# jhbastek/PhysicsInformedDiffusionModels

Hardware: AMD Instinct MI355X
Metric: training samples/sec (UNet+PDE-residual step), 64x64 Darcy (higher is better)
Workload: dtype f32

## Files before the change

physicsinformeddiffusionmodels_amd/csrc/k_attn.hip:

```cpp
#include "pidm_launch.h"

namespace pidm {

static const int DH = 32;

__device__ __forceinline__ float fexp(float x) { return __expf(x); }

__global__ void __launch_bounds__(256) la_kstats_kernel(const float* __restrict__ qkv, int N, int HD, int nseg,
                                                        float* __restrict__ kpart, float* __restrict__ kstat) {
  __shared__ float sm[4][64], ssum[4][64];
  const int b = blockIdx.y, seg = blockIdx.z, tid = threadIdx.x, cl = tid & 63, rl = tid >> 6;
  const int j = blockIdx.x * 64 + cl;
  const int per = (N + nseg - 1) / nseg;
  const int n_lo = seg * per, n_hi = (n_lo + per < N) ? n_lo + per : N;
  float m = -3.0e38f, s = 0.f;
  if (j < HD) {
    const float* base = qkv + (size_t)b * N * 3 * HD + HD + j;
    int n = n_lo + rl;
    for (; n + 28 < n_hi; n += 32) {
      float v[8];
#pragma unroll
      for (int u = 0; u < 8; ++u) v[u] = base[(size_t)(n + 4 * u) * 3 * HD];
      float gm = v[0];
#pragma unroll
// ... 700 lines not shown
    for (int it = 0; it < 4; ++it) {
      const f32x4 v = *reinterpret_cast<const f32x4*>(tb + (trow + 8 * it) * kLaTileLd + tcol);
      *reinterpret_cast<f32x4*>(orow + (size_t)(trow + 8 * it) * 3 * HD + tcol) = v;
    }
  }
}

static const int kLaDkvLds = 32 * 33 + 96;
__global__ void __launch_bounds__(256, 3) la_bwd_dkdv_kernel(const float* __restrict__ qkv, const float* __restrict__ kstat,
                                                             const float* __restrict__ dctx, const float* __restrict__ rowdot,
                                                             float* __restrict__ dqkv, int N, int heads) {
  HIP_DYNAMIC_SHARED(float, sm)
  const int HD = heads * DH;
  const int tid = threadIdx.x, lane = tid & 63, wave = tid >> 6, half = lane >> 5, l31 = lane & 31;
  const size_t pblk = (size_t)blockIdx.x * 128;
  const int b = (int)(pblk / N);
  const size_t pa = pblk + wave * 32 + l31;
  const float invN = 1.f / (float)N;
  for (int i = tid; i < heads * 1024; i += 256)
    sm[(i >> 10) * kLaDkvLds + ((i & 1023) >> 5) * 33 + (i & 31)] = dctx[(size_t)b * heads * 1024 + i];
  for (int i = tid; i < heads * 32; i += 256) {
    float* hs = sm + (i >> 5) * kLaDkvLds + 1056;
    hs[i & 31] = rowdot[(size_t)b * heads * 32 + i];
    hs[32 + (i & 31)] = kstat[((size_t)b * HD + i) * 2];
    hs[64 + (i & 31)] = kstat[((size_t)b * HD + i) * 2 + 1];
  }
  __syncthreads();
  float* tb = sm + heads * kLaDkvLds + wave * (32 * kLaTileLd);
  const float* rowK = qkv + pa * 3 * HD + HD;
  f32x4 n_k[4], n_v[4], n_k4[4];
#pragma unroll
  for (int j = 0; j < 4; ++j) {
    n_k[j] = *reinterpret_cast<const f32x4*>(rowK + 16 * half + 4 * j);
    n_v[j] = *reinterpret_cast<const f32x4*>(rowK + HD + 16 * half + 4 * j);
    n_k4[j] = *reinterpret_cast<const f32x4*>(rowK + 8 * j + 4 * half);
  }
  for (int h = 0; h < heads; ++h) {
    const float* sd = sm + h * kLaDkvLds;
    const float* srd = sd + 1056;
    const float* skm = srd + 32;
    const float* skis = srd + 64;
    f32x4 a_k[4], a_v[4], k4[4];
#pragma unroll
    for (int j = 0; j < 4; ++j) { a_k[j] = n_k[j]; a_v[j] = n_v[j]; k4[j] = n_k4[j]; }
    if (h + 1 < heads) {
      const float* rn = rowK + (h + 1) * DH;
#pragma unroll
      for (int j = 0; j < 4; ++j) {
        n_k[j] = *reinterpret_cast<const f32x4*>(rn + 16 * half + 4 * j);
        n_v[j] = *reinterpret_cast<const f32x4*>(rn + HD + 16 * half + 4 * j);
        n_k4[j] = *reinterpret_cast<const f32x4*>(rn + 8 * j + 4 * half);
      }
    }
    f32x16 acc2, acc3;
    for (int r = 0; r < 16; ++r) { acc2[r] = 0.f; acc3[r] = 0.f; }
#pragma unroll
    for (int j = 0; j < 4; ++j) {
#pragma unroll
      for (int c = 0; c < 4; ++c) {
        const int kk = 16 * half + 4 * j + c;
        acc2 = __builtin_amdgcn_mfma_f32_32x32x2f32(sd[l31 * 33 + kk], a_v[j][c], acc2, 0, 0, 0);
        const float pB = fexp(a_k[j][c] - skm[kk]) * skis[kk];
        acc3 = __builtin_amdgcn_mfma_f32_32x32x2f32(sd[kk * 33 + l31], pB, acc3, 0, 0, 0);
      }
    }
    f32x4 o_k[4], o_v[4];
#pragma unroll
    for (int j = 0; j < 4; ++j) {
#pragma unroll
      for (int c = 0; c < 4; ++c) {
        const int d = 8 * j + 4 * half + c;
        const float P = fexp(k4[j][c] - skm[d]) * skis[d];
        o_k[j][c] = P * (acc2[4 * j + c] * invN - srd[d]);
        o_v[j][c] = acc3[4 * j + c] * invN;
      }
    }
    float* ok = dqkv + (pblk + wave * 32) * 3 * HD + HD + h * DH;
    const int trow = lane >> 3, tcol = 4 * (lane & 7);
#pragma unroll
    for (int which = 0; which < 2; ++which) {
      __builtin_amdgcn_wave_barrier();
#pragma unroll
      for (int j = 0; j < 4; ++j) *reinterpret_cast<f32x4*>(tb + l31 * kLaTileLd + 8 * j + 4 * half) = which ? o_v[j] : o_k[j];
      __builtin_amdgcn_wave_barrier();
#pragma unroll
      for (int it = 0; it < 4; ++it) {
        const f32x4 v = *reinterpret_cast<const f32x4*>(tb + (trow + 8 * it) * kLaTileLd + tcol);
        *reinterpret_cast<f32x4*>(ok + (size_t)(trow + 8 * it) * 3 * HD + which * HD + tcol) = v;
      }
    }
  }
}

template <bool BWD>
__global__ void __launch_bounds__(256) mid_attn_kernel(const float* __restrict__ qkv, const float* __restrict__ dO,
                                                       float* __restrict__ out,
                                                       int N, int heads, float scale) {
  HIP_DYNAMIC_SHARED(float, smem)
  float (*sq)[33] = reinterpret_cast<float (*)[33]>(smem);
  float (*sk)[33] = reinterpret_cast<float (*)[33]>(smem + (size_t)N * 33);
  float (*sv)[33] = reinterpret_cast<float (*)[33]>(smem + (size_t)2 * N * 33);
  float (*sdo)[33] = reinterpret_cast<float (*)[33]>(smem + (size_t)3 * N * 33);
  float* sS_ = smem + (size_t)4 * N * 33;
  float* sdS_ = sS_ + (size_t)N * (N + 1);
  const int LS = N + 1;
#define sS(i, j) sS_[(i) * LS + (j)]
#define sdS(i, j) sdS_[(i) * LS + (j)]
  const int HD = heads * DH;
  const int bh = blockIdx.x, b = bh / heads, h = bh % heads, tid = threadIdx.x;
  for (int e = tid; e < N * 32; e += 256) {
    const int n = e >> 5, d = e & 31;
    const float* row = qkv + ((size_t)b * N + n) * 3 * HD + h * DH + d;
    sq[n][d] = row[0] * scale;
    sk[n][d] = row[HD];
    sv[n][d] = row[2 * HD];
    if (BWD) sdo[n][d] = dO[((size_t)b * N + n) * HD + h * DH + d];
  }
  __syncthreads();
  for (int e = tid; e < N * N; e += 256) {
    const int i = e / N, j = e % N;
    float s = 0.f;
#pragma unroll
    for (int d = 0; d < 32; ++d) s = fmaf(sq[i][d], sk[j][d], s);
    sS(i, j) = s;
  }
  __syncthreads();
  if (tid < N) {
    float m = -3.0e38f;
    for (int j = 0; j < N; ++j) m = fmaxf(m, sS(tid, j));
    float s = 0.f;
    for (int j = 0; j < N; ++j) {
      const float ex = fexp(sS(tid, j) - m);
      sS(tid, j) = ex;
      s += ex;
    }
    const float inv = 1.f / s;
    for (int j = 0; j < N; ++j) sS(tid, j) *= inv;
  }
  __syncthreads();
  if (!BWD) {
    for (int e = tid; e < N * 32; e += 256) {
      const int i = e >> 5, d = e & 31;
      float o = 0.f;
      for (int j = 0; j < N; ++j) o = fmaf(sS(i, j), sv[j][d], o);
      out[((size_t)b * N + i) * HD + h * DH + d] = o;
    }
    return;
  }
  for (int e = tid; e < N * 32; e += 256) {
    const int j = e >> 5, d = e & 31;
    float o = 0.f;
    for (int i = 0; i < N; ++i) o = fmaf(sS(i, j), sdo[i][d], o);
    out[((size_t)b * N + j) * 3 * HD + 2 * HD + h * DH + d] = o;
  }
  __syncthreads();
  for (int e = tid; e < N * N; e += 256) {
    const int i = e / N, j = e % N;
    float s = 0.f;
#pragma unroll
    for (int d = 0; d < 32; ++d) s = fmaf(sdo[i][d], sv[j][d], s);
    sdS(i, j) = s;
  }
  __syncthreads();
  if (tid < N) {
    float dot = 0.f;
    for (int j = 0; j < N; ++j) dot = fmaf(sdS(tid, j), sS(tid, j), dot);
    for (int j = 0; j < N; ++j) sdS(tid, j) = sS(tid, j) * (sdS(tid, j) - dot);
  }
  __syncthreads();
  for (int e = tid; e < N * 32; e += 256) {
    const int i = e >> 5, d = e & 31;
    float a = 0.f, c = 0.f;
    for (int j = 0; j < N; ++j) {
      a = fmaf(sdS(i, j), sk[j][d], a);
      c = fmaf(sdS(j, i), sq[j][d], c);
    }
    out[((size_t)b * N + i) * 3 * HD + h * DH + d] = a * scale;
    out[((size_t)b * N + i) * 3 * HD + HD + h * DH + d] = c;
  }
}

#undef sS
#undef sdS

template <bool BWD>
__global__ void __launch_bounds__(256) mid_attn64_kernel(const float* __restrict__ qkv, const float* __restrict__ dO,
                                                         float* __restrict__ out, int heads, float scale) {
  constexpr int N = 64, LS = 65;
  HIP_DYNAMIC_SHARED(float, smem)
  float (*sq)[33] = reinterpret_cast<float (*)[33]>(smem);
  float (*sk)[33] = reinterpret_cast<float (*)[33]>(smem + (size_t)N * 33);
  float (*sv)[33] = reinterpret_cast<float (*)[33]>(smem + (size_t)2 * N * 33);
  float (*sdo)[33] = reinterpret_cast<float (*)[33]>(smem + (size_t)3 * N * 33);
  float* sS_ = smem + (size_t)4 * N * 33;
  float* sdS_ = sS_ + (size_t)N * LS;
  const int HD = heads * DH;
  const int bh = blockIdx.x, b = bh / heads, h = bh % heads, tid = threadIdx.x;
  const int lane = tid & 63, half = lane >> 5, l31 = lane & 31, wave = __builtin_amdgcn_readfirstlane(tid >> 6);
  for (int e = tid; e < N * 32; e += 256) {
    const int n = e >> 5, d = e & 31;
    const float* row = qkv + ((size_t)b * N + n) * 3 * HD + h * DH + d;
    sq[n][d] = row[0] * scale;
    sk[n][d] = row[HD];
    sv[n][d] = row[2 * HD];
    if (BWD) sdo[n][d] = dO[((size_t)b * N + n) * HD + h * DH + d];
  }
  __syncthreads();
  const int ti = wave >> 1, tj = wave & 1;
  {
    f32x16 acc;
    for (int r = 0; r < 16; ++r) acc[r] = 0.f;
#pragma unroll
    for (int s2 = 0; s2 < 16; ++s2)
      acc = __builtin_amdgcn_mfma_f32_32x32x2f32(sq[32 * ti + l31][2 * s2 + half], sk[32 * tj + l31][2 * s2 + half], acc, 0, 0, 0);
#pragma unroll
    for (int r = 0; r < 16; ++r) sS_[(32 * ti + (r & 3) + 8 * (r >> 2) + 4 * half) * LS + 32 * tj + l31] = acc[r];
  }
  __syncthreads();
  {
    const int row = tid >> 2, c0 = (tid & 3) * 16;
    float* pr = sS_ + row * LS + c0;
    float m = pr[0];
#pragma unroll
    for (int j = 1; j < 16; ++j) m = fmaxf(m, pr[j]);
    m = fmaxf(m, pidm_quad_xor1(m));
    m = fmaxf(m, pidm_quad_xor2(m));
    float ex[16], sum = 0.f;
#pragma unroll
    for (int j = 0; j < 16; ++j) { ex[j] = fexp(pr[j] - m); sum += ex[j]; }
    sum += pidm_quad_xor1(sum);
    sum += pidm_quad_xor2(sum);
    const float inv = 1.f / sum;
#pragma unroll
    for (int j = 0; j < 16; ++j) pr[j] = ex[j] * inv;
  }
  __syncthreads();
  if (!BWD) {
    if (wave < 2) {
      f32x16 acc;
      for (int r = 0; r < 16; ++r) acc[r] = 0.f;
#pragma unroll 8
      for (int s2 = 0; s2 < 32; ++s2)
        acc = __builtin_amdgcn_mfma_f32_32x32x2f32(sS_[(32 * wave + l31) * LS + 2 * s2 + half], sv[2 * s2 + half][l31], acc, 0, 0, 0);
#pragma unroll
      for (int r = 0; r < 16; ++r)
        out[((size_t)b * N + 32 * wave + (r & 3) + 8 * (r >> 2) + 4 * half) * HD + h * DH + l31] = acc[r];
    }
    return;
  }
  {
    f32x16 acc;
    for (int r = 0; r < 16; ++r) acc[r] = 0.f;
#pragma unroll
    for (int s2 = 0; s2 < 16; ++s2)
      acc = __builtin_amdgcn_mfma_f32_32x32x2f32(sdo[32 * ti + l31][2 * s2 + half], sv[32 * tj + l31][2 * s2 + half], acc, 0, 0, 0);
#pragma unroll
    for (int r = 0; r < 16; ++r) sdS_[(32 * ti + (r & 3) + 8 * (r >> 2) + 4 * half) * LS + 32 * tj + l31] = acc[r];
  }
  if (wave < 2) {
    f32x16 acc;
    for (int r = 0; r < 16; ++r) acc[r] = 0.f;
#pragma unroll 8
    for (int s2 = 0; s2 < 32; ++s2)
      acc = __builtin_amdgcn_mfma_f32_32x32x2f32(sS_[(2 * s2 + half) * LS + 32 * wave + l31], sdo[2 * s2 + half][l31], acc, 0, 0, 0);
#pragma unroll
    for (int r = 0; r < 16; ++r)
      out[((size_t)b * N + 32 * wave + (r & 3) + 8 * (r >> 2) + 4 * half) * 3 * HD + 2 * HD + h * DH + l31] = acc[r];
  }
  __syncthreads();
  {
    const int row = tid >> 2, c0 = (tid & 3) * 16;
    const float* pp = sS_ + row * LS + c0;
    float* pd = sdS_ + row * LS + c0;
    float dot = 0.f;
#pragma unroll
    for (int j = 0; j < 16; ++j) dot = fmaf(pd[j], pp[j], dot);
    dot += pidm_quad_xor1(dot);
    dot += pidm_quad_xor2(dot);
#pragma unroll
    for (int j = 0; j < 16; ++j) pd[j] = pp[j] * (pd[j] - dot);
  }
  __syncthreads();
  {
    const int t = wave & 1;
    f32x16 acc;
    for (int r = 0; r < 16; ++r) acc[r] = 0.f;
    if (wave < 2) {
#pragma unroll 8
      for (int s2 = 0; s2 < 32; ++s2)
        acc = __builtin_amdgcn_mfma_f32_32x32x2f32(sdS_[(32 * t + l31) * LS + 2 * s2 + half], sk[2 * s2 + half][l31], acc, 0, 0, 0);
    } else {
#pragma unroll 8
      for (int s2 = 0; s2 < 32; ++s2)
        acc = __builtin_amdgcn_mfma_f32_32x32x2f32(sdS_[(2 * s2 + half) * LS + 32 * t + l31], sq[2 * s2 + half][l31], acc, 0, 0, 0);
    }
    const float f = wave < 2 ? scale : 1.f;
    const size_t col = (wave < 2 ? 0 : HD) + h * DH + l31;
#pragma unroll
    for (int r = 0; r < 16; ++r)
      out[((size_t)b * N + 32 * t + (r & 3) + 8 * (r >> 2) + 4 * half) * 3 * HD + col] = acc[r] * f;
  }
}

static int la_nsplit(int N) {
  int ns = N / 512;
  if (ns < 1) ns = 1;
  if (ns > 8) ns = 8;
  return ns;
}
static int la_kseg(int N) {
  int s = N / 256;
  if (s < 1) s = 1;
  if (s > 16) s = 16;
  return s;
}
size_t la_scratch_floats(int B, int N, int heads) {
  const size_t a = (size_t)B * la_kseg(N) * heads * DH * 2, b = (size_t)B * heads * la_nsplit(N) * 1024;
  return a + b + (size_t)heads * DH * 128 + 64;
}

int launch_la_forward(const float* qkv, float* kstat, float* ctx, float* attn, float* qstat, int B, int N, int heads,
                      float* scratch, hipStream_t st) {
  const int HD = heads * DH;
  const float scale = 0.17677669529663687f;
  const int nseg = la_kseg(N), NS = la_nsplit(N);
  float* kpart = scratch;
  float* dpart = scratch + (size_t)B * nseg * HD * 2;
  hipLaunchKernelGGL(la_kstats_kernel, dim3(cdiv(HD, 64), B, nseg), dim3(256), 0, st, qkv, N, HD, nseg, kpart, nseg == 1 ? kstat : nullptr);
  PIDM_CHECK_LAUNCH("la_kstats_kernel");
  if (nseg > 1) {
    hipLaunchKernelGGL(la_kstats_final_kernel, dim3(cdiv(B * HD, 256)), dim3(256), 0, st, kpart, B, HD, nseg, kstat);
    PIDM_CHECK_LAUNCH("la_kstats_final_kernel");
  }
  hipLaunchKernelGGL(HIP_KERNEL_NAME(la_nreduce_kernel<0>), dim3(B * heads, NS), dim3(256), 0, st, qkv, kstat, nullptr, nullptr,
                     dpart, N, heads, scale, NS == 1 ? ctx : nullptr, nullptr, 1.f / (float)N);
  PIDM_CHECK_LAUNCH("la_context");
  if (NS > 1) {
    hipLaunchKernelGGL(HIP_KERNEL_NAME(la_nreduce_final_kernel<0>), dim3(B * heads), dim3(256), 0, st, dpart, nullptr, ctx, nullptr, NS,
                       1.f / (float)N);
    PIDM_CHECK_LAUNCH("la_context_final");
  }
  const size_t npix = (size_t)B * N;
  if (N % 32 == 0)
    hipLaunchKernelGGL(HIP_KERNEL_NAME(la_out_kernel<true>), dim3((unsigned)((npix + 127) / 128), (npix + 127) / 128 < 1024 ? heads : 1), dim3(256), 0, st, qkv, ctx, attn,
                       qstat, N, heads, npix, scale);
  else
    hipLaunchKernelGGL(HIP_KERNEL_NAME(la_out_kernel<false>), dim3((unsigned)((npix + 127) / 128), (npix + 127) / 128 < 1024 ? heads : 1), dim3(256), 0, st, qkv, ctx, attn,
                       qstat, N, heads, npix, scale);
  PIDM_CHECK_LAUNCH("la_out_kernel");
  return 0;
}

int launch_la_backward(const float* qkv, const float* kstat, const float* qstat, const float* ctx, const float* dA, float* dctx,
                       float* rowdot, float* dqkv, int B, int N, int heads, float* scratch, hipStream_t st) {
  const float scale = 0.17677669529663687f;
  const int NS = la_nsplit(N);
  float* dpart = scratch;
  hipLaunchKernelGGL(HIP_KERNEL_NAME(la_nreduce_kernel<1>), dim3(B * heads, NS), dim3(256), 0, st, qkv, qstat, dA, ctx, dpart, N, heads,
                     scale, NS == 1 ? dctx : nullptr, rowdot, 1.f);
  PIDM_CHECK_LAUNCH("la_dctx");
  if (NS > 1) {
    hipLaunchKernelGGL(HIP_KERNEL_NAME(la_nreduce_final_kernel<1>), dim3(B * heads), dim3(256), 0, st, dpart, ctx, dctx, rowdot, NS, 1.f);
    PIDM_CHECK_LAUNCH("la_dctx_final");
  }
  if (N % 32 == 0 && N >= 64) {
    const size_t npix = (size_t)B * N;
    int ppb = N % 128 == 0 ? 128 : (N % 64 == 0 ? 64 : 32);
    (void)npix;
    if (const char* pe = knob("PIDM_LA_PPB")) { const int v = atoi(pe); if ((v == 32 || v == 64 || v == 128) && N % v == 0) ppb = v; }
    PIDM_PROF_NAME("la_bwd_pix_mfma_kernel");
    hipLaunchKernelGGL(la_bwd_pix_mfma_kernel, dim3((unsigned)((size_t)B * N / ppb), heads), dim3(2 * ppb), 0, st, qkv, kstat, qstat, ctx,
                       dctx, rowdot, dA, dqkv, N, heads, scale, ppb);
  } else {
    hipLaunchKernelGGL(la_bwd_pix_kernel, dim3(cdiv(N, 256), B * heads), dim3(256), 0, st, qkv, kstat, qstat, ctx, dctx, rowdot,
                       dA, dqkv, N, heads, scale);
  }
  PIDM_CHECK_LAUNCH("la_bwd_pix_kernel");
  return 0;
}

bool la_fused_ok(int N, int heads, int Cout, int ld_dy) {
  const bool off = knob("PIDM_NO_LA_FUSED") != nullptr;
  return !off && N % 128 == 0 && (Cout == 32 || Cout == 64 || Cout == 128) && (ld_dy & 3) == 0 && heads >= 1 && heads <= 14;
}
int launch_la_forward_fused(const float* qkv, float* kstat, float* ctx, float* qstat, const float* w_out, const float* bias,
                            const float* resid, float* y, int Cout, int B, int N, int heads, float* scratch, hipStream_t st) {
  if (!la_fused_ok(N, heads, Cout, Cout)) return fail("fused attention forward: N=%d Cout=%d not eligible", N, Cout);
  const int HD = heads * DH;
  const float scale = 0.17677669529663687f;
  const int nseg = la_kseg(N), NS = la_nsplit(N);
  float* kpart = scratch;
  float* dpart = scratch + (size_t)B * nseg * HD * 2;
  hipLaunchKernelGGL(la_kstats_kernel, dim3(cdiv(HD, 64), B, nseg), dim3(256), 0, st, qkv, N, HD, nseg, kpart, nseg == 1 ? kstat : nullptr);
  PIDM_CHECK_LAUNCH("la_kstats_kernel");
  if (nseg > 1) {
    hipLaunchKernelGGL(la_kstats_final_kernel, dim3(cdiv(B * HD, 256)), dim3(256), 0, st, kpart, B, HD, nseg, kstat);
    PIDM_CHECK_LAUNCH("la_kstats_final_kernel");
  }
  hipLaunchKernelGGL(HIP_KERNEL_NAME(la_nreduce_kernel<0>), dim3(B * heads, NS), dim3(256), 0, st, qkv, kstat, nullptr, nullptr,
                     dpart, N, heads, scale, NS == 1 ? ctx : nullptr, nullptr, 1.f / (float)N);
  PIDM_CHECK_LAUNCH("la_context");
  if (NS > 1) {
    hipLaunchKernelGGL(HIP_KERNEL_NAME(la_nreduce_final_kernel<0>), dim3(B * heads), dim3(256), 0, st, dpart, nullptr, ctx, nullptr, NS,
                       1.f / (float)N);
    PIDM_CHECK_LAUNCH("la_context_final");
  }
  float* wt = dpart + (size_t)B * heads * NS * 1024;
  hipLaunchKernelGGL(la_wt_kernel, dim3(cdiv(Cout * HD, 256)), dim3(256), 0, st, w_out, wt, Cout, HD);
  PIDM_CHECK_LAUNCH("la_wt_kernel");
  const dim3 grid((unsigned)((size_t)B * N / 128));
  if (Cout == 32)
    hipLaunchKernelGGL(HIP_KERNEL_NAME(la_out_proj_kernel<1>), grid, dim3(256), 0, st, qkv, ctx, wt, bias, resid, y, qstat, N, heads, scale);
  else if (Cout == 64)
    hipLaunchKernelGGL(HIP_KERNEL_NAME(la_out_proj_kernel<2>), grid, dim3(256), 0, st, qkv, ctx, wt, bias, resid, y, qstat, N, heads, scale);
  else
    hipLaunchKernelGGL(HIP_KERNEL_NAME(la_out_proj_kernel<4>), grid, dim3(256), 0, st, qkv, ctx, wt, bias, resid, y, qstat, N, heads, scale);
  PIDM_CHECK_LAUNCH("la_out_proj_kernel");
  return 0;
}

bool la_fused_pays(int B, int N) {
  const char* mw = knob("PIDM_LA_FUSED_MIN_WGS");
  const long min_wgs = mw ? atol(mw) : 256;
  return (long)B * N / 128 >= min_wgs;
}
size_t la_fused_scratch_floats(int B, int N, int heads, int Cout) {
  return (size_t)B * heads * la_nsplit(N) * (Cout / 32) * 1024 + 64;
}
int launch_la_backward_fused(const float* qkv, const float* kstat, const float* qstat, const float* ctx, const float* dy, int ld_dy,
                             const float* w_out, int Cout, float* dctx, float* rowdot, float* dqkv, float* dwpart, int B, int N,
                             int heads, float* scratch, hipStream_t st) {
  if (!la_fused_ok(N, heads, Cout, ld_dy)) return fail("fused attention backward: N=%d Cout=%d not eligible", N, Cout);
  const float scale = 0.17677669529663687f;
  const int NS = la_nsplit(N);
  float* gpart = scratch;
  const dim3 grid(B * heads, NS);
#define PIDM_LA_G(NT_)                                                                                                        \
  {                                                                                                                           \
    hipLaunchKernelGGL(HIP_KERNEL_NAME(la_g_kernel<NT_>), grid, dim3(256), 0, st, qkv, qstat, dy, ld_dy, gpart, N, heads, scale); \
    PIDM_CHECK_LAUNCH("la_g_kernel");                                                                                         \
    hipLaunchKernelGGL(HIP_KERNEL_NAME(la_g_final_kernel<NT_>), dim3(B * heads), dim3(256), 0, st, gpart, ctx, w_out, dctx,    \
                       rowdot, dwpart, NS, heads);                                                                            \
    PIDM_CHECK_LAUNCH("la_g_final_kernel");                                                                                   \
  }
  if (Cout == 32) PIDM_LA_G(1)
  else if (Cout == 64) PIDM_LA_G(2)
  else PIDM_LA_G(4)
#undef PIDM_LA_G
  const dim3 gridp((unsigned)((size_t)B * N / 128));
  static bool attr_done = false;
  if (!attr_done) {
    (void)hipFuncSetAttribute(reinterpret_cast<const void*>(&la_bwd_dq_kernel), hipFuncAttributeMaxDynamicSharedMemorySize, 96 * 1024);
    (void)hipFuncSetAttribute(reinterpret_cast<const void*>(&la_bwd_dkdv_kernel), hipFuncAttributeMaxDynamicSharedMemorySize, 96 * 1024);
    attr_done = true;
  }
  hipLaunchKernelGGL(la_bwd_dq_kernel, gridp, dim3(256), ((size_t)heads * 1056 + 4 * 32 * kLaTileLd) * sizeof(float), st, qkv, qstat, ctx, dy, ld_dy, w_out, Cout,
                     dqkv, N, heads, scale);
  PIDM_CHECK_LAUNCH("la_bwd_dq_kernel");
  hipLaunchKernelGGL(la_bwd_dkdv_kernel, gridp, dim3(256), ((size_t)heads * kLaDkvLds + 4 * 32 * kLaTileLd) * sizeof(float), st, qkv, kstat, dctx, rowdot, dqkv, N,
                     heads);
  PIDM_CHECK_LAUNCH("la_bwd_dkdv_kernel");
  return 0;
}

int launch_mid_attn(const float* qkv, const float* dO, float* out, int B, int N, int heads, bool bwd, hipStream_t st) {
  if (N > 64) return fail("mid attention: %d tokens > 64", N);
  const float scale = 0.17677669529663687f;
  const size_t lds = ((size_t)4 * N * 33 + (size_t)2 * N * (N + 1)) * sizeof(float);
  static bool attr_done = false;
  if (!attr_done) {
    (void)hipFuncSetAttribute(reinterpret_cast<const void*>(&mid_attn_kernel<true>), hipFuncAttributeMaxDynamicSharedMemorySize, 96 * 1024);
    (void)hipFuncSetAttribute(reinterpret_cast<const void*>(&mid_attn_kernel<false>), hipFuncAttributeMaxDynamicSharedMemorySize, 96 * 1024);
    attr_done = true;
  }
  const bool mfma_off = [] { const char* e = knob("PIDM_MID_ATTN_MFMA"); return e && !atoi(e); }();
  if (N == 64 && !mfma_off) {
    static bool attr64 = false;
    if (!attr64) {
      (void)hipFuncSetAttribute(reinterpret_cast<const void*>(&mid_attn64_kernel<true>), hipFuncAttributeMaxDynamicSharedMemorySize, 96 * 1024);
      (void)hipFuncSetAttribute(reinterpret_cast<const void*>(&mid_attn64_kernel<false>), hipFuncAttributeMaxDynamicSharedMemorySize, 96 * 1024);
      attr64 = true;
    }
    if (bwd) hipLaunchKernelGGL(HIP_KERNEL_NAME(mid_attn64_kernel<true>), dim3(B * heads), dim3(256), lds, st, qkv, dO, out, heads, scale);
    else hipLaunchKernelGGL(HIP_KERNEL_NAME(mid_attn64_kernel<false>), dim3(B * heads), dim3(256), lds, st, qkv, dO, out, heads, scale);
    PIDM_CHECK_LAUNCH("mid_attn64_kernel");
    return 0;
  }
  if (bwd)
    hipLaunchKernelGGL(HIP_KERNEL_NAME(mid_attn_kernel<true>), dim3(B * heads), dim3(256), lds, st, qkv, dO, out, N, heads, scale);
  else
    hipLaunchKernelGGL(HIP_KERNEL_NAME(mid_attn_kernel<false>), dim3(B * heads), dim3(256), lds, st, qkv, dO, out, N, heads, scale);
  PIDM_CHECK_LAUNCH("mid_attn_kernel");
  return 0;
}

}

extern "C" size_t pidm_linear_attention_ws(int B, int N, int heads) {
  return ((size_t)B * heads * (1024 + 32) + pidm::la_scratch_floats(B, N, heads)) * sizeof(float);
}
extern "C" int pidm_linear_attention_forward(const float* qkv, float* out, float* kstat, float* ctx, float* qstat, int B, int N,
                                             int heads, void* workspace, void* stream) {
  if (!qkv || !out || !kstat || !ctx || !qstat || !workspace || B < 1 || N < 1 || heads < 1)
    return pidm::fail("linear attention: bad arguments");
  float* scratch = reinterpret_cast<float*>(workspace) + (size_t)B * heads * (1024 + 32);
  return pidm::launch_la_forward(qkv, kstat, ctx, out, qstat, B, N, heads, scratch, reinterpret_cast<hipStream_t>(stream));
}
extern "C" int pidm_linear_attention_backward(const float* qkv, const float* kstat, const float* qstat, const float* ctx,
                                              const float* d_out, float* dqkv, int B, int N, int heads, void* workspace,
                                              void* stream) {
  if (!qkv || !kstat || !qstat || !ctx || !d_out || !dqkv || !workspace || B < 1 || N < 1 || heads < 1)
    return pidm::fail("linear attention backward: bad arguments");
  float* dctx = reinterpret_cast<float*>(workspace);
  float* rowdot = dctx + (size_t)B * heads * 1024;
  float* scratch = rowdot + (size_t)B * heads * 32;
  return pidm::launch_la_backward(qkv, kstat, qstat, ctx, d_out, dctx, rowdot, dqkv, B, N, heads, scratch,
                                  reinterpret_cast<hipStream_t>(stream));
}
extern "C" size_t pidm_linear_attention_out_backward_ws(int B, int N, int heads, int Cout) {
  return ((size_t)B * heads * (1024 + 32) + (size_t)B * Cout * heads * 32 + pidm::la_fused_scratch_floats(B, N, heads, Cout)) *
         sizeof(float);
}
extern "C" int pidm_linear_attention_out_backward(const float* qkv, const float* kstat, const float* qstat, const float* ctx,
                                                  const float* d_y, int ld_dy, const float* w_out, int Cout, float* dqkv,
                                                  float* dw_out, int B, int N, int heads, void* workspace, void* stream) {
  if (!qkv || !kstat || !qstat || !ctx || !d_y || !w_out || !dqkv || !dw_out || !workspace || B < 1)
    return pidm::fail("fused attention backward: bad arguments");
  const int HD = heads * 32;
  float* dctx = reinterpret_cast<float*>(workspace);
  float* rowdot = dctx + (size_t)B * heads * 1024;
  float* dwpart = rowdot + (size_t)B * heads * 32;
  float* scratch = dwpart + (size_t)B * Cout * HD;
  hipStream_t st = reinterpret_cast<hipStream_t>(stream);
  if (pidm::launch_la_backward_fused(qkv, kstat, qstat, ctx, d_y, ld_dy, w_out, Cout, dctx, rowdot, dqkv, dwpart, B, N, heads,
                                     scratch, st))
    return -1;
  return pidm::launch_split_reduce(dwpart, dw_out, nullptr, nullptr, B, Cout, HD, 1, Cout, HD, st);
}
extern "C" int pidm_linear_attention_out_forward(const float* qkv, const float* w_out, const float* bias, const float* residual,
                                                 float* y, int Cout, float* kstat, float* ctx, float* qstat, int B, int N,
                                                 int heads, void* workspace, void* stream) {
  if (!qkv || !w_out || !y || !kstat || !ctx || !qstat || !workspace || B < 1) return pidm::fail("fused attention forward: bad arguments");
  float* scratch = reinterpret_cast<float*>(workspace) + (size_t)B * heads * (1024 + 32);
  return pidm::launch_la_forward_fused(qkv, kstat, ctx, qstat, w_out, bias, residual, y, Cout, B, N, heads, scratch,
                                       reinterpret_cast<hipStream_t>(stream));
}
```

Baseline: 7933.

## Fuse linear-attention forward and backward into single per-head LDS-resident kernels

For small spatial sizes (N between 64 and 256, multiple of 32), forward and backward linear attention each run as one kernel per (batch, head). The kernel stages K/V (or Q/K/dA) into LDS and computes key stats, context, query softmax and output with MFMA inside one block. This replaces the chain of separate stats, reduce, finalize and output launches and their global scratch round-trips. In exchange, parallelism drops to B*heads blocks that need large dynamic LDS, which can limit occupancy. The backward kernel also no longer writes dctx and rowdot to global memory.

```diff
diff --git a/physicsinformeddiffusionmodels_amd/csrc/k_attn.hip b/physicsinformeddiffusionmodels_amd/csrc/k_attn.hip
--- a/physicsinformeddiffusionmodels_amd/csrc/k_attn.hip
+++ b/physicsinformeddiffusionmodels_amd/csrc/k_attn.hip
@@ -1026,6 +1026,330 @@
   }
 }
 
+__device__ __forceinline__ int la_one_swz(int row, int piece) { return row * 32 + 4 * (piece ^ ((row >> 1) & 7)); }
+template <bool SWZ>
+__device__ __forceinline__ void la_one_stage(const float* __restrict__ src, size_t ld, float* __restrict__ dst, int N, int wave,
+                                             int nw, int lane) {
+  for (int c = wave; c < N / 8; c += nw) {
+    const int row = 8 * c + (lane >> 3);
+    const int piece = SWZ ? ((lane & 7) ^ ((row >> 1) & 7)) : (lane & 7);
+    pidm_glds_b128(src + (size_t)row * ld + 4 * piece, dst + 256 * c);
+  }
+}
+#ifdef PIDM_HAVE_ROW_SHL
+__device__ __forceinline__ float la_half_sum(float x) {
+  for (int off = 1; off < 32; off <<= 1) x += __shfl_xor(x, off);
+  return x;
+}
+#else
+template <int CTRL>
+__device__ __forceinline__ float la_dpp(float v) {
+  return __builtin_bit_cast(float, __builtin_amdgcn_update_dpp(0, __builtin_bit_cast(int, v), CTRL, 0xF, 0xF, true));
+}
+__device__ __forceinline__ float la_half_sum(float x) {
+  x += pidm_quad_xor1(x);
+  x += pidm_quad_xor2(x);
+  x += la_dpp<0x1B >(la_dpp<0x141 >(x));
+  x += la_dpp<0x141>(la_dpp<0x140 >(x));
+  const unsigned u = __builtin_bit_cast(unsigned, x);
+  const auto sw = __builtin_amdgcn_permlane16_swap(u, u, false, false);
+  return x + __builtin_bit_cast(float, (__lane_id() & 16) ? sw[0] : sw[1]);
+}
+#endif
+static int la_one_waves(int N) { return N > 128 ? 8 : 4; }
+static size_t la_fwd_one_lds(int N) { return ((size_t)64 * N + 1024 + 4 * 64 + 64) * sizeof(float); }
+static size_t la_bwd_one_lds(int N) { return ((size_t)98 * N + 4096 + 2 * 32 * kLaTileLd + 96) * sizeof(float); }
+
+__global__ void __launch_bounds__(512) la_fwd_one_kernel(const float* __restrict__ qkv, float* __restrict__ kstat,
+                                                         float* __restrict__ ctx, float* __restrict__ attn,
+                                                         float* __restrict__ qstat, int N, int heads, float scale, float alpha) {
+  HIP_DYNAMIC_SHARED(float, lds)
+  float* sk = lds;
+  float* sv = sk + N * 32;
+  float* sctx = sv + N * 32;
+  float* spm = sctx + 1024;
+  float* sps = spm + 128;
+  float* scm = sps + 128;
+  float* scis = scm + 32;
+  float* red = lds;
+  const int bh = blockIdx.x, b = bh / heads, h = bh % heads;
+  const int HD = heads * DH;
+  const int tid = threadIdx.x, lane = tid & 63, half = lane >> 5, l31 = lane & 31;
+  const int wave = __builtin_amdgcn_readfirstlane(tid >> 6), nw = blockDim.x >> 6, nt = blockDim.x;
+  const float* q0 = qkv + (size_t)b * N * 3 * HD + h * DH;
+  la_one_stage<false>(q0 + HD, 3 * HD, sk, N, wave, nw, lane);
+  la_one_stage<false>(q0 + 2 * HD, 3 * HD, sv, N, wave, nw, lane);
+  const bool tile = wave * 32 < N;
+  float qv[16];
+  if (tile) {
+    const float* qp = q0 + (size_t)(wave * 32 + l31) * 3 * HD + 16 * half;
+#pragma unroll
+    for (int k = 0; k < 4; ++k) {
+      const float4 v = *reinterpret_cast<const float4*>(qp + 4 * k);
+      qv[4 * k] = v.x; qv[4 * k + 1] = v.y; qv[4 * k + 2] = v.z; qv[4 * k + 3] = v.w;
+    }
+  }
+  PIDM_WAIT_VMEM();
+  __syncthreads();
+  if (tid < 128) {
+    const int cl = tid & 31, rl = tid >> 5;
+    float m = -3.0e38f, s = 0.f;
+    const float* base = sk + cl;
+    int n = rl;
+    for (; n + 28 < N; n += 32) {
+      float v[8];
+#pragma unroll
+      for (int u = 0; u < 8; ++u) v[u] = base[(n + 4 * u) * 32];
+      float gm = v[0];
+#pragma unroll
+      for (int u = 1; u < 8; ++u) gm = fmaxf(gm, v[u]);
+      const float mn = fmaxf(m, gm);
+      float gs = 0.f;
+#pragma unroll
+      for (int u = 0; u < 8; ++u) gs += fexp(v[u] - mn);
+      s = s * fexp(m - mn) + gs;
+      m = mn;
+    }
+    for (; n < N; n += 4) {
+      const float v = base[n * 32];
+      const float mn = fmaxf(m, v);
+      s = s * fexp(m - mn) + fexp(v - mn);
+      m = mn;
+    }
+    spm[rl * 32 + cl] = m;
+    sps[rl * 32 + cl] = s;
+  }
+  __syncthreads();
+  if (tid < 32) {
+    const float M = fmaxf(fmaxf(spm[tid], spm[32 + tid]), fmaxf(spm[64 + tid], spm[96 + tid]));
+    float S = 0.f;
+    for (int r = 0; r < 4; ++r) S += sps[r * 32 + tid] * fexp(spm[r * 32 + tid] - M);
+    const float is = 1.f / S;
+    kstat[((size_t)b * HD + h * DH + tid) * 2] = M;
+    kstat[((size_t)b * HD + h * DH + tid) * 2 + 1] = is;
+    scm[tid] = M;
+    scis[tid] = is;
+  }
+  __syncthreads();
+  {
+    const float cm = scm[l31], cis = scis[l31];
+    f32x16 acc;
+    for (int r = 0; r < 16; ++r) acc[r] = 0.f;
+    const int per = N / 4;
+    for (int n0 = wave * per; wave < 4 && n0 < (wave + 1) * per; n0 += 8) {
+      float av[4], bvv[4];
+#pragma unroll
+      for (int u = 0; u < 4; ++u) {
+        av[u] = sk[(n0 + 2 * u + half) * 32 + l31];
+        bvv[u] = sv[(n0 + 2 * u + half) * 32 + l31];
+      }
+#pragma unroll
+      for (int u = 0; u < 4; ++u) {
+        const float a = fexp(av[u] - cm) * cis;
+        acc = __builtin_amdgcn_mfma_f32_32x32x2f32(a, bvv[u], acc, 0, 0, 0);
+      }
+    }
+    __syncthreads();
+    if (wave < 4) {
+      for (int r = 0; r < 16; ++r) {
+        const int row = (r & 3) + 8 * (r >> 2) + 4 * half;
+        red[wave * 1024 + row * 32 + l31] = acc[r];
+      }
+    }
+    __syncthreads();
+    for (int e = tid; e < 1024; e += nt) {
+      const float v = ((red[e] + red[1024 + e]) + (red[2048 + e] + red[3072 + e])) * alpha;
+      ctx[(size_t)bh * 1024 + e] = v;
+      sctx[e] = v;
+    }
+    __syncthreads();
+  }
+  if (tile) {
+    const size_t pw = (size_t)b * N + wave * 32, p = pw + l31;
+    float m = -3.0e38f;
+#pragma unroll
+    for (int k = 0; k < 16; ++k) m = fmaxf(m, qv[k]);
+    m = fmaxf(m, pidm_other_half(m));
+    float s = 0.f;
+#pragma unroll
+    for (int k = 0; k < 16; ++k) {
+      qv[k] = fexp(qv[k] - m);
+      s += qv[k];
+    }
+    s += pidm_other_half(s);
+    const float inv = 1.f / s;
+    if (half == 0) {
+      qstat[(p * heads + h) * 2] = m;
+      qstat[(p * heads + h) * 2 + 1] = inv;
+    }
+    f32x16 acc;
+    for (int r = 0; r < 16; ++r) acc[r] = 0.f;
+#pragma unroll
+    for (int s2 = 0; s2 < 16; ++s2) {
+      const float a = qv[s2] * inv * scale;
+      const float bv = sctx[(16 * half + s2) * 32 + l31];
+      acc = __builtin_amdgcn_mfma_f32_32x32x2f32(a, bv, acc, 0, 0, 0);
+    }
+#pragma unroll
+    for (int r = 0; r < 16; ++r) {
+      const int row = (r & 3) + 8 * (r >> 2) + 4 * half;
+      attn[(pw + row) * HD + h * DH + l31] = acc[r];
+    }
+  }
+}
+
+__global__ void __launch_bounds__(512) la_bwd_one_kernel(const float* __restrict__ qkv, const float* __restrict__ kstat,
+                                                         const float* __restrict__ qstat, const float* __restrict__ ctx,
+                                                         const float* __restrict__ dA, float* __restrict__ dqkv, int N, int heads,
+                                                         float scale) {
+  HIP_DYNAMIC_SHARED(float, lds)
+  float* sq = lds;
+  float* sk = sq + N * 32;
+  float* sda = sk + N * 32;
+  float* red = sda + N * 32;
+  float* sc = red + 4096;
+  float* sd = sc + 32 * kLaTileLd;
+  float* srd = sd + 32 * kLaTileLd;
+  float* skm = srd + 32;
+  float* skis = skm + 32;
+  float* sqs = skis + 32;
+  const int bh = blockIdx.x, b = bh / heads, h = bh % heads;
+  const int HD = heads * DH;
+  const int tid = threadIdx.x, lane = tid & 63, half = lane >> 5, l31 = lane & 31;
+  const int wave = __builtin_amdgcn_readfirstlane(tid >> 6), nw = blockDim.x >> 6, nt = blockDim.x;
+  const float* q0 = qkv + (size_t)b * N * 3 * HD + h * DH;
+  const float* dA0 = dA + (size_t)b * N * HD + h * DH;
+  const float invN = 1.f / (float)N;
+  la_one_stage<false>(q0, 3 * HD, sq, N, wave, nw, lane);
+  la_one_stage<true>(dA0, HD, sda, N, wave, nw, lane);
+  la_one_stage<true>(q0 + HD, 3 * HD, sk, N, wave, nw, lane);
+  const bool tile = wave * 32 < N;
+  f32x4 a_v[4];
+  if (tile) {
+#pragma unroll
+    for (int j = 0; j < 4; ++j)
+      a_v[j] = *reinterpret_cast<const f32x4*>(q0 + (size_t)(wave * 32 + l31) * 3 * HD + 2 * HD + 16 * half + 4 * j);
+  }
+  {
+    const int nc = 1024 / nt;
+    float c4[4];
+#pragma unroll
+    for (int k = 0; k < 4; ++k) c4[k] = k < nc ? ctx[(size_t)bh * 1024 + tid + nt * k] : 0.f;
+    float2 qs2 = make_float2(0.f, 0.f), ks2 = make_float2(0.f, 0.f);
+    if (tid < N) qs2 = *reinterpret_cast<const float2*>(qstat + (((size_t)b * N + tid) * heads + h) * 2);
+    if (tid < 32) ks2 = *reinterpret_cast<const float2*>(kstat + ((size_t)b * HD + h * DH + tid) * 2);
+#pragma unroll
+    for (int k = 0; k < 4; ++k) {
+      const int e = tid + nt * k;
+      if (k < nc) sc[(e >> 5) * kLaTileLd + (e & 31)] = c4[k];
+    }
+    if (tid < N) {
+      sqs[2 * tid] = qs2.x;
+      sqs[2 * tid + 1] = qs2.y;
+    }
+    if (tid < 32) {
+      skm[tid] = ks2.x;
+      skis[tid] = ks2.y;
+    }
+  }
+  PIDM_WAIT_VMEM();
+  __syncthreads();
+  {
+    f32x16 acc;
+    for (int r = 0; r < 16; ++r) acc[r] = 0.f;
+    const int per = N / 4;
+    for (int n0 = wave * per; wave < 4 && n0 < (wave + 1) * per; n0 += 8) {
+      float av[4], bvv[4];
+      float2 qs[4];
+#pragma unroll
+      for (int u = 0; u < 4; ++u) {
+        const int n = n0 + 2 * u + half;
+        av[u] = sq[n * 32 + l31];
+        bvv[u] = sda[la_one_swz(n, l31 >> 2) + (l31 & 3)];
+        qs[u] = make_float2(sqs[2 * n], sqs[2 * n + 1]);
+      }
+#pragma unroll
+      for (int u = 0; u < 4; ++u) {
+        const float a = fexp(av[u] - qs[u].x) * qs[u].y * scale;
+        acc = __builtin_amdgcn_mfma_f32_32x32x2f32(a, bvv[u], acc, 0, 0, 0);
+      }
+    }
+    if (wave < 4) {
+      for (int r = 0; r < 16; ++r) {
+        const int row = (r & 3) + 8 * (r >> 2) + 4 * half;
+        red[wave * 1024 + row * 32 + l31] = acc[r];
+      }
+    }
+    __syncthreads();
+    for (int e = tid; e < 1024; e += nt)
+      sd[(e >> 5) * kLaTileLd + (e & 31)] = ((red[e] + red[1024 + e]) + (red[2048 + e] + red[3072 + e])) * 1.f;
+    __syncthreads();
+    for (int e = tid; e < 1024; e += nt) red[e] = sd[(e >> 5) * kLaTileLd + (e & 31)] * sc[(e >> 5) * kLaTileLd + (e & 31)];
+    __syncthreads();
+    if (tid < 32) {
+      float sacc = 0.f;
+      for (int j = 0; j < 32; ++j) sacc += red[tid * 32 + j];
+      srd[tid] = sacc;
+    }
+    __syncthreads();
+  }
+  if (tile) {
+    const int na = wave * 32 + l31;
+    f32x4 a_dA[4], a_k[4], b_c[4], b_d[4], k_m[4], k_is[4];
+#pragma unroll
+    for (int j = 0; j < 4; ++j) {
+      a_dA[j] = *reinterpret_cast<const f32x4*>(sda + la_one_swz(na, 4 * half + j));
+      a_k[j] = *reinterpret_cast<const f32x4*>(sk + la_one_swz(na, 4 * half + j));
+      b_c[j] = *reinterpret_cast<const f32x4*>(sc + l31 * kLaTileLd + 16 * half + 4 * j);
+      b_d[j] = *reinterpret_cast<const f32x4*>(sd + l31 * kLaTileLd + 16 * half + 4 * j);
+      k_m[j] = *reinterpret_cast<const f32x4*>(skm + 16 * half + 4 * j);
+      k_is[j] = *reinterpret_cast<const f32x4*>(skis + 16 * half + 4 * j);
+    }
+    f32x16 acc1, acc2, acc3;
+    for (int r = 0; r < 16; ++r) { acc1[r] = 0.f; acc2[r] = 0.f; acc3[r] = 0.f; }
+#pragma unroll
+    for (int j = 0; j < 4; ++j) {
+#pragma unroll
+      for (int c = 0; c < 4; ++c) {
+        const int s = 4 * j + c, kk = 16 * half + s;
+        acc1 = __builtin_amdgcn_mfma_f32_32x32x2f32(a_dA[j][c], b_c[j][c], acc1, 0, 0, 0);
+        acc2 = __builtin_amdgcn_mfma_f32_32x32x2f32(a_v[j][c], b_d[j][c], acc2, 0, 0, 0);
+        const float pA = fexp(a_k[j][c] - k_m[j][c]) * k_is[j][c];
+        acc3 = __builtin_amdgcn_mfma_f32_32x32x2f32(pA, sd[kk * kLaTileLd + l31], acc3, 0, 0, 0);
+      }
+    }
+    const float km = skm[l31], kis = skis[l31], rd = srd[l31];
+#pragma unroll
+    for (int r = 0; r < 16; ++r) {
+      const int n = wave * 32 + (r & 3) + 8 * (r >> 2) + 4 * half;
+      const float qm = sqs[2 * n], qis = sqs[2 * n + 1];
+      const float qs = fexp(sq[n * 32 + l31] - qm) * qis;
+      const float dot = la_half_sum(qs * acc1[r]);
+      float* o = dqkv + ((size_t)b * N + n) * 3 * HD + h * DH + l31;
+      o[0] = scale * qs * (acc1[r] - dot);
+      const float P = fexp(sk[la_one_swz(n, l31 >> 2) + (l31 & 3)] - km) * kis;
+      o[HD] = P * (acc2[r] * invN - rd);
+      o[2 * HD] = acc3[r] * invN;
+    }
+  }
+}
+
+static const size_t kLaOneMaxLds = 160 * 1024 - 256;
+static bool la_one_ok(int N) {
+  const char* e = knob("PIDM_LA_ONE");
+  if (e && !atoi(e)) return false;
+  return N % 32 == 0 && N >= 64 && N <= 256 && la_bwd_one_lds(N) <= kLaOneMaxLds && la_fwd_one_lds(N) <= kLaOneMaxLds;
+}
+static int la_one_attr() {
+  static bool attr_done = false;
+  if (!attr_done) {
+    if (hipFuncSetAttribute(reinterpret_cast<const void*>(&la_fwd_one_kernel), hipFuncAttributeMaxDynamicSharedMemorySize, (int)kLaOneMaxLds) != hipSuccess ||
+        hipFuncSetAttribute(reinterpret_cast<const void*>(&la_bwd_one_kernel), hipFuncAttributeMaxDynamicSharedMemorySize, (int)kLaOneMaxLds) != hipSuccess)
+      return fail("one-launch linear attention: cannot raise the dynamic LDS limit");
+    attr_done = true;
+  }
+  return 0;
+}
 static int la_nsplit(int N) {
   int ns = N / 512;
   if (ns < 1) ns = 1;
@@ -1047,6 +1371,14 @@
                       float* scratch, hipStream_t st) {
   const int HD = heads * DH;
   const float scale = 0.17677669529663687f;
+  if (la_one_ok(N)) {
+    if (la_one_attr()) return -1;
+    PIDM_PROF_NAME("la_fwd_one_kernel");
+    hipLaunchKernelGGL(la_fwd_one_kernel, dim3(B * heads), dim3(64 * la_one_waves(N)), la_fwd_one_lds(N), st, qkv, kstat, ctx, attn, qstat, N, heads, scale,
+                       1.f / (float)N);
+    PIDM_CHECK_LAUNCH("la_fwd_one_kernel");
+    return 0;
+  }
   const int nseg = la_kseg(N), NS = la_nsplit(N);
   float* kpart = scratch;
   float* dpart = scratch + (size_t)B * nseg * HD * 2;
@@ -1078,6 +1410,14 @@
 int launch_la_backward(const float* qkv, const float* kstat, const float* qstat, const float* ctx, const float* dA, float* dctx,
                        float* rowdot, float* dqkv, int B, int N, int heads, float* scratch, hipStream_t st) {
   const float scale = 0.17677669529663687f;
+  if (la_one_ok(N)) {
+    if (la_one_attr()) return -1;
+    PIDM_PROF_NAME("la_bwd_one_kernel");
+    hipLaunchKernelGGL(la_bwd_one_kernel, dim3(B * heads), dim3(64 * la_one_waves(N)), la_bwd_one_lds(N), st, qkv, kstat, qstat, ctx, dA, dqkv, N, heads,
+                       scale);
+    PIDM_CHECK_LAUNCH("la_bwd_one_kernel");
+    return 0;
+  }
   const int NS = la_nsplit(N);
   float* dpart = scratch;
   hipLaunchKernelGGL(HIP_KERNEL_NAME(la_nreduce_kernel<1>), dim3(B * heads, NS), dim3(256), 0, st, qkv, qstat, dA, ctx, dpart, N, heads,
```

Result: no change. 7987 (median of 6 runs) (+0.7%).
